# thekingofkings/embedding

Measured on AMD Instinct MI355X. Metric: SGNS training edges/sec, higher is better.
Workload: dtype f32

## Files before the change

### embedding_amd/_native.py

```python
import ctypes as C
import os

_HERE = os.path.dirname(os.path.abspath(__file__))
LIB_PATH = os.path.join(_HERE, "libdge.so")

DGE_OK, DGE_ERR_ARG, DGE_ERR_RANGE, DGE_ERR_TOPK, DGE_ERR_CAP, DGE_ERR_STATE, DGE_ERR_DEVICE, DGE_ERR_IO = range(8)


class DgeError(RuntimeError):
    def __init__(self, code, msg):
        super().__init__("libdge error %d: %s" % (code, msg))
        self.code = code


class TrainConfig(C.Structure):
    _fields_ = [
        ("dim", C.c_int32), ("window", C.c_int32), ("negative", C.c_int32), ("min_count", C.c_int32),
        ("epochs", C.c_int32), ("workers", C.c_int32), ("alpha", C.c_float), ("min_alpha", C.c_float),
        ("seed", C.c_uint64), ("table_size", C.c_int64), ("n_vertices", C.c_int32), ("update_policy", C.c_int32),
        ("use_hs", C.c_int32), ("reserved", C.c_int32),
    ]


class TrainStats(C.Structure):
# ... 55 lines not shown
    "dge_names_add": (_int, [_vp, _vp, _i64]),
    "dge_names_count": (_int, [_vp, _P(_i64)]),
    "dge_names_cstrs": (_int, [_vp, _P(_vp)]),
    "dge_names_free": (None, [_vp]),
    "dge_walks_from_seq_text": (_int, [_int, _vp, _i64, _vp, _int, _P(_vp), _P(SeqInfo)]),
    "dge_walks_from_seq_files": (_int, [_int, _vp, _i32, _vp, _int, _P(_vp), _P(SeqInfo)]),
    "dge_walks_to_seq_text": (_int, [_vp, _i64, _i64, _vp, _int, _vp, _i64, _P(_i64), _P(SeqOutInfo)]),
    "dge_walks_write_seq": (_int, [_vp, _i64, _i64, _vp, _int, C.c_char_p, _int, _P(SeqOutInfo)]),
    "dge_walks_to_host": (_int, [_vp, _vp, _i64]),
    "dge_walks_info": (_int, [_vp, _P(_i64), _P(_i32), _P(_vp)]),
    "dge_walks_add_position_prefix": (_int, [_vp, _i32]),
    "dge_walks_free": (None, [_vp]),
    "dge_count_tokens": (_int, [_vp, _i64, _i64, _i32, _vp]),
    "dge_model_create": (_int, [_int, _P(TrainConfig), _vp, _P(_vp)]),
    "dge_model_set_stream": (_int, [_vp, _vp]),
    "dge_model_train": (_int, [_vp, _vp, _i64, _i64, _i64, _i32, _i64, _dbl, _i64]),
    "dge_train_sgns": (_int, [_int, _vp, _i64, _i32, _P(TrainConfig), _P(_vp)]),
    "dge_train_sgns_device": (_int, [_vp, _P(TrainConfig), _P(_vp)]),
    "dge_model_walk_and_train": (_int, [_vp, _vp, _vp, _i64, _i64, _i64, _i64, _i32, _i64, _dbl, _i64]),
    "dge_model_vectors": (_int, [_vp, _P(_vp), _P(_vp), _P(_i64), _P(_i32)]),
    "dge_model_syn1neg": (_int, [_vp, _P(_vp)]),
    "dge_model_syn1": (_int, [_vp, _P(_vp), _P(_i64)]),
    "dge_model_huffman": (_int, [_vp, _P(_vp), _P(_vp), _P(_vp)]),
    "dge_model_counts": (_int, [_vp, _P(_vp)]),
    "dge_model_table": (_int, [_vp, _P(_vp), _P(_i64)]),
    "dge_model_stats": (_int, [_vp, _P(TrainStats)]),
    "dge_model_row_rates": (_int, [_vp, _P(C.c_double), _P(C.c_double), _P(C.c_double), _P(C.c_double)]),
    "dge_model_table_placement": (_int, [_vp, _i32, _vp, _vp, _vp]),
    "dge_model_table_runs": (_int, [_vp, _vp, _vp]),
    "dge_model_tune_placement": (_int, [_vp, _vp, _i64, _i64, _i32, _vp, _vp, _vp]),
    "dge_model_placement_search": (_int, [_vp, _vp, _vp, _vp, _vp]),
    "dge_model_reset_stats": (_int, [_vp]),
    "dge_model_schedule": (_int, [_vp, _P(_i32), _P(_i64), _P(_i32)]),
    "dge_model_kernel": (_int, [_vp, C.c_char_p, _i32]),
    "dge_model_lock_stats": (_int, [_vp, _P(_i64), _P(_i64), _P(_i64)]),
    "dge_model_score_pairs": (_int, [_vp, _vp, _vp, _i64, _vp]),
    "dge_model_eval_links": (_int, [_vp, _vp, _i64, _i64, _i32, C.c_uint64, _P(EvalResult)]),
    "dge_model_eval_sgns": (_int, [_vp, _vp, _i64, _i64, C.c_uint64, _P(EvalResult)]),
    "dge_write_vec": (_int, [_vp, _vp, C.c_char_p, _int]),
    "dge_model_free": (None, [_vp]),
    "dge_model_set_partition": (_int, [_vp, _i32, _i32, _i32]),
    "dge_model_partition_floats": (_int, [_vp, _i32, _P(_i64)]),
    "dge_model_export_partition": (_int, [_vp, _int, _i32, _i32, _vp]),
    "dge_model_import_partition": (_int, [_vp, _int, _i32, _i32, _vp]),
    "dge_model_export_partition_async": (_int, [_vp, _int, _i32, _i32, _vp, _vp]),
    "dge_model_import_partition_async": (_int, [_vp, _int, _i32, _i32, _vp, _vp]),
    "dge_model_stream": (_int, [_vp, _P(_vp)]),
    "dge_host_sync_count": (_int, [_P(_i64)]),
    "dge_model_sync_size": (_int, [_vp, _P(_i64)]),
    "dge_model_snapshot": (_int, [_vp]),
    "dge_model_export_delta": (_int, [_vp, _vp]),
    "dge_model_import_delta": (_int, [_vp, _vp, C.c_float]),
    "dge_comm_unique_id": (_int, [_vp]),
    "dge_comm_create": (_int, [_P(_vp), _vp, _int, _int, _int]),
    "dge_comm_free": (None, [_vp]),
    "dge_model_allreduce_deltas": (_int, [_vp, _vp]),
    "dge_model_ring_pass": (_int, [_vp, _vp, _i32]),
    "dge_model_gather_table": (_int, [_vp, _vp, _int]),
    "dge_set_tuning": (_int, [_i32, _i64]),
    "dge_get_tuning": (_int, [_i32, _vp]),
    "dge_ndcg_at_k": (_int, [_int, _vp, _i32, _vp, _i32, _i32, _i32, _P(_dbl), _P(_dbl)]),
    "dge_knn_cosine": (_int, [_int, _vp, _i32, _i32, _i32, _vp, _vp, _P(_dbl)]),
    "dge_vectors_from_vec_text": (_int, [_int, _vp, _i64, _int, _vp, _int, _P(_vp), _P(VecInfo)]),
    "dge_vectors_from_vec_files": (_int, [_int, _vp, _i32, _int, _vp, _int, _P(_vp), _P(VecInfo)]),
    "dge_vectors_from_host": (_int, [_int, _vp, _i64, _i32, _vp, _P(_vp)]),
    "dge_vectors_info": (_int, [_vp, _P(_i64), _P(_i32), _P(_vp), _P(_vp)]),
# ... 50 lines not shown
```

### embedding_amd/csrc/sgns.hip

```cpp
#include <hipcub/hipcub.hpp>
#include <math.h>
#include <stdlib.h>
#include <string.h>

#include <algorithm>
#include <limits>
#include <string>

#include "dge_algos.h"
#include "dge_internal.h"
#include "sgns_kernels.h"
#include "sgns_model.h"

std::atomic<int64_t> g_dge_tuning[DGE_TUNE_COUNT];
namespace { struct TuningInit { TuningInit() { for (auto& k : g_dge_tuning) k.store(-1); } } g_tuning_init; }
std::atomic<int64_t> g_dge_host_syncs{0};
extern "C" int dge_host_sync_count(int64_t* n) {
    if (!n) DGE_FAIL(DGE_ERR_ARG, "dge_host_sync_count: null output");
    *n = g_dge_host_syncs.load(std::memory_order_relaxed);
    return DGE_OK;
}
extern "C" int dge_set_tuning(int32_t knob, int64_t value) {
    if (knob < 0 || knob >= DGE_TUNE_COUNT) DGE_FAIL(DGE_ERR_ARG, "dge_set_tuning: unknown knob %d", knob);
    g_dge_tuning[knob] = value < 0 ? -1 : value;
// ... 554 lines not shown
    dge_model* m = const_cast<dge_model*>(mc);
    if (!m || !out) DGE_FAIL(DGE_ERR_ARG, "dge_model_stats: null argument");
    int rc = dge_drain_events(m);
    if (rc) return rc;
    unsigned long long c[4] = {0, 0, 0, 0};
    DGE_HIP(hipMemcpy(c, m->d_counters, sizeof(c), hipMemcpyDeviceToHost));
    out->pairs = (int64_t)c[0]; out->words = (int64_t)c[1];
    out->kernel_ms = m->kernel_ms; out->walk_kernel_ms = m->walk_ms; out->launches = m->launches;
    if (c[3]) {
        DGE_HIP(hipMemsetAsync(m->d_counters + 3, 0, sizeof(unsigned long long), m->stream));
        DGE_HIP(hipStreamSynchronize(m->stream));
        DGE_FAIL(DGE_ERR_STATE, "a training launch was ended by its watchdog: %llu workers waited for row locks beyond the launch's time budget and left their walks untrained "
                 "(update_policy %d on this vocabulary: use 0 (auto) or 7)", c[3], m->cfg.update_policy);
    }
    return DGE_OK;
}

extern "C" int dge_model_table_runs(const dge_model* m, int32_t* n_runs, int32_t* n_exceptions) {
    if (!m) DGE_FAIL(DGE_ERR_ARG, "dge_model_table_runs: null model");
    if (n_runs) *n_runs = m->n_runs;
    if (n_exceptions) *n_exceptions = m->n_exc;
    return DGE_OK;
}

extern "C" int dge_model_schedule(const dge_model* m, int32_t* update_policy, int64_t* workers, int32_t* hot_rows) {
    if (!m) DGE_FAIL(DGE_ERR_ARG, "dge_model_schedule: null model");
    if (!m->has_plan) DGE_FAIL(DGE_ERR_STATE, "dge_model_schedule: nothing has been trained yet");
    if (update_policy) *update_policy = m->last_plan.reported_policy();
    if (workers) *workers = m->last_plan.workers;
    if (hot_rows) *hot_rows = m->last_plan.hot_rows;
    return DGE_OK;
}

extern "C" int dge_model_lock_stats(const dge_model* mc, int64_t* pairs_put_back, int64_t* rounds_short, int64_t* rounds) {
    dge_model* m = const_cast<dge_model*>(mc);
    if (!m) DGE_FAIL(DGE_ERR_ARG, "dge_model_lock_stats: null model");
    DGE_HIP(hipSetDevice(m->device));
    DGE_HIP(hipStreamSynchronize(m->stream));
    unsigned long long c[3] = {0, 0, 0};
    DGE_HIP(hipMemcpy(c, m->d_counters + 4, sizeof(c), hipMemcpyDeviceToHost));
    if (pairs_put_back) *pairs_put_back = (int64_t)c[0];
    if (rounds_short) *rounds_short = (int64_t)c[1];
    if (rounds) *rounds = (int64_t)c[2];
    return DGE_OK;
}

extern "C" int dge_model_kernel(const dge_model* m, char* buf, int32_t cap) {
    if (!m || !buf || cap <= 0) DGE_FAIL(DGE_ERR_ARG, "dge_model_kernel: bad argument");
    if (!m->has_plan) DGE_FAIL(DGE_ERR_STATE, "dge_model_kernel: nothing has been trained yet");
    snprintf(buf, (size_t)cap, "%s", m->last_plan.kernel_name().c_str());
    return DGE_OK;
}

extern "C" int dge_model_reset_stats(dge_model* m) {
    if (!m) DGE_FAIL(DGE_ERR_ARG, "dge_model_reset_stats: null model");
    int rc = dge_drain_events(m);
    if (rc) return rc;
    DGE_HIP(hipMemsetAsync(m->d_counters, 0, 2 * sizeof(unsigned long long), m->stream));
    DGE_HIP(hipMemsetAsync(m->d_counters + 4, 0, 3 * sizeof(unsigned long long), m->stream));
    DGE_HIP(hipStreamSynchronize(m->stream));
    m->kernel_ms = 0; m->walk_ms = 0; m->launches = 0;
    return DGE_OK;
}

extern "C" int dge_model_set_partition(dge_model* m, int32_t n_parts, int32_t ctx_part, int32_t tgt_part) {
    if (!m) DGE_FAIL(DGE_ERR_ARG, "dge_model_set_partition: null model");
// ... 7 lines not shown
```

### embedding_amd/csrc/sgns_kernels.h

```cpp
#pragma once
#include <hip/hip_runtime.h>
#include <stdint.h>

#include "dge_algos.h"
#include "dge_internal.h"
#include "sgns_plan.h"

#define EXP_TABLE_SIZE 1000
#define MAX_EXP 6
#define NEG_BATCH 5

struct TrainParams {
    const int32_t* sen; const int64_t* len; const int64_t* wb;
    float* syn0; float* syn1neg;
    int32_t acc_rows, acc_drain;
    const uint4* ctab;
    const double* run_base; const uint32_t* run_row; const uint32_t* exc_slot; const int32_t* exc_row;
    int32_t n_runs, n_exc;
    double T_inv;
    const float* exp_table;
    int64_t n_rows; int32_t L, W, K, stride;
    int32_t D;
    int64_t V, T;
    uint64_t T_magic, W_magic;
// ... 1150 lines not shown
            l1.v[q].x += neu.v[q].x; l1.v[q].y += neu.v[q].y; l1.v[q].z += neu.v[q].z; l1.v[q].w += neu.v[q].w;
        }
        if (HOTMIX && (last < hot_rows || p.syn0_free)) {
            if (use_mb) lk_post<DCH>(s_mb, s_mb_flag, wk, n_posts, 2, lane == 0 ? last : -1, 1.0f, neu, lane);
            else rowA_atomic_axpy<DCH>(syn0, last, lane, 1.0f, neu);
        } else {
            rowA_store<DCH, 16, BIG>(l1, syn0, last, lane);
            row_commit_wait(STRICT ? row_probe_lines(syn0, last, lane, DCH * 2) : 0.f);
            if (lane == 14) row_unlock<STRICT>(locks0, last);
        }
        my_pairs++;
        if (PART) {
            pair_mask &= pair_mask - 1ull;
            c = first_bit_from(pair_mask, 0, c_hi + 1);
        } else {
            c++;
            if (c == i) c++;
        }
    }
    LK_CLOSE_CENTRE();
    if (pend_row >= 0 && !flushA_blocking<DCH, STRICT, BIG, HOTMIX>(syn1neg, locks1, pend_row, my_dh + (cur_buf ^ 1) * DCH * 64 + lane, lane, hot_rows, WD ? &s_deadline : nullptr)) LK_GIVE_UP();
#undef LK_TOK
#undef LK_POSITIVE
#undef LK_CLOSE_CENTRE
#undef LK_GIVE_UP
    if (lane == 0) {
        if (my_pairs) atomicAdd(&p.counters[0], my_pairs);
        if (my_words) atomicAdd(&p.counters[1], my_words);
        if (PART) { atomicAdd(&p.counters[4], (unsigned long long)n_aborted); atomicAdd(&p.counters[5], (unsigned long long)n_short); atomicAdd(&p.counters[6], (unsigned long long)n_rounds); }
        if (use_mb) __hip_atomic_fetch_add(&s_mb_done, 1, __ATOMIC_RELEASE, __HIP_MEMORY_SCOPE_WORKGROUP);
    }
}

#define HSW_NQ (DCH <= 2 ? 6 : 3)
template <int DCH>
__device__ __forceinline__ void hot_addA(float* s_hot, int* s_cnt, int slot, int drain, const TableView& t, int32_t row, int lane, const Row<DCH>& x) {
    float* a = s_hot + slot * (DCH * 64) + 4 * lane;
#pragma unroll
    for (int c = 0; c < DCH; c++) {
        atomicAdd(a + c * 64 + 0, x.v[c].x); atomicAdd(a + c * 64 + 1, x.v[c].y); atomicAdd(a + c * 64 + 2, x.v[c].z); atomicAdd(a + c * 64 + 3, x.v[c].w);
    }
    int n = 0;
    if (lane == 0) n = atomicAdd(&s_cnt[slot], 1) + 1;
    n = __shfl(n, 0, 16);
    if (n % drain == 0) {
        float* e = s_hot + slot * (DCH * 64) + lane;
        float* gp = t.base + (size_t)row * (t.row_bytes / 4) + lane;
#pragma unroll
        for (int c = 0; c < DCH; c++)
#pragma unroll
            for (int m = 0; m < 4; m++) {
                if ((uint32_t)(c * 64 + 16 * m + lane) >= t.valid) continue;
                const float v = atomicExch(e + c * 64 + 16 * m, 0.f);
                if (v != 0.f) atomicAdd(gp + c * 64 + 16 * m, v);
            }
    }
}
template <int DCH>
__device__ __forceinline__ void row_add(Row<DCH>& y, const Row<DCH>& x) {
#pragma unroll
    for (int c = 0; c < DCH; c++) { y.v[c].x += x.v[c].x; y.v[c].y += x.v[c].y; y.v[c].z += x.v[c].z; y.v[c].w += x.v[c].w; }
}
__device__ __forceinline__ int hsw_n_copies(const TrainParams& p, int32_t nd) {
    int r = 1;
#pragma unroll
    for (int k = 1; k < HS_REP; k++) r += nd >= p.hs_rep_thr[k] ? 1 : 0;
// ... 477 lines not shown
            if (pl.hs) {
                if (pl.part) hipLaunchKernelGGL((k_sgns_train<DCH, 2, BIG, true, true>), g, b, pl.shmem, st, p);
                else hipLaunchKernelGGL((k_sgns_train<DCH, 2, BIG, true, false>), g, b, pl.shmem, st, p);
            } else if (pl.part) hipLaunchKernelGGL((k_sgns_train<DCH, 2, BIG, false, true>), g, b, 0, st, p);
            else hipLaunchKernelGGL((k_sgns_train<DCH, 2, BIG, false, false>), g, b, 0, st, p);
            break;
        case TrainForm::HsCentre:
            if constexpr (DCH <= 4 && !BIG) {
                if (!pl.nlock) hipLaunchKernelGGL((k_sgns_train_hsw<DCH, false, 3>), g, b, pl.shmem, st, p);
                else if (pl.waves == 3) {
                    if (pl.head) hipLaunchKernelGGL((k_sgns_train_hsw<DCH, true, 3, true>), g, b, pl.shmem, st, p);
                    else hipLaunchKernelGGL((k_sgns_train_hsw<DCH, true, 3>), g, b, pl.shmem, st, p);
                } else if constexpr (DCH <= 2) {
                    if (pl.head) {
                        (void)hipFuncSetAttribute((const void*)k_sgns_train_hsw<DCH, true, 7, true>, hipFuncAttributeMaxDynamicSharedMemorySize, (int)pl.shmem);
                        hipLaunchKernelGGL((k_sgns_train_hsw<DCH, true, 7, true>), g, b, pl.shmem, st, p);
                    } else {
                        (void)hipFuncSetAttribute((const void*)k_sgns_train_hsw<DCH, true, 7>, hipFuncAttributeMaxDynamicSharedMemorySize, (int)pl.shmem);
                        hipLaunchKernelGGL((k_sgns_train_hsw<DCH, true, 7>), g, b, pl.shmem, st, p);
                    }
                }
            }
            break;
        case TrainForm::Locked:
            if (pl.hotmix) {
                if (pl.part) hipLaunchKernelGGL((k_sgns_train_locked<DCH, false, BIG, true, true>), g, b, 0, st, p);
                else hipLaunchKernelGGL((k_sgns_train_locked<DCH, false, BIG, true, false>), g, b, 0, st, p);
            } else if (pl.part) {
                if (pl.wdog) hipLaunchKernelGGL((k_sgns_train_locked<DCH, false, BIG, false, true, true>), g, b, 0, st, p);
                else hipLaunchKernelGGL((k_sgns_train_locked<DCH, false, BIG, false, true>), g, b, 0, st, p);
            } else if (pl.strict) {
                if (pl.wdog) hipLaunchKernelGGL((k_sgns_train_locked<DCH, true, BIG, false, false, true>), g, b, 0, st, p);
                else hipLaunchKernelGGL((k_sgns_train_locked<DCH, true, BIG, false, false>), g, b, 0, st, p);
            } else {
                if (pl.wdog) hipLaunchKernelGGL((k_sgns_train_locked<DCH, false, BIG, false, false, true>), g, b, 0, st, p);
                else hipLaunchKernelGGL((k_sgns_train_locked<DCH, false, BIG, false, false>), g, b, 0, st, p);
            }
            break;
        default: break;
    }
}
template <int DCH>
static inline void launch_train(const TrainParams& p, const TrainPlan& pl, hipStream_t st) {
    if (pl.big) launch_train_b<DCH, true>(p, pl, st);
    else launch_train_b<DCH, false>(p, pl, st);
}
```

### embedding_amd/csrc/sgns_plan.h

```cpp
#pragma once
#include <math.h>
#include <stdarg.h>
#include <stdint.h>
#include <stdio.h>

#include <algorithm>
#include <string>
#include <vector>

#include "../../include/dge.h"

#define HS_REP 16
#define HS_REP_NODES 64
#define HS_REP_ROWS ((HS_REP - 1) * HS_REP_NODES)
#ifndef DGE_LOCKED_WAVES
#define DGE_LOCKED_WAVES 3
#endif
#ifndef DGE_HOTMIX_WAVES
#define DGE_HOTMIX_WAVES 3
#endif
#ifndef DGE_HS_WAVES
#define DGE_HS_WAVES 3
#endif

static inline double dge_expected_pairs_per_walk(int L, int W) {
    double e = 0.0;
    for (int i = 0; i < L; i++)
        for (int r = 1; r <= W; r++) e += (double)(std::min(L - 1, i + r) - std::max(0, i - r)) / (double)W;
    return e;
}

struct ScheduleStats {
    int64_t V = 0;
    int32_t D = 0, stride = 0;
    int64_t total_words = 0;
    double neg_norm = 1.0;
    double neg_collision = 1.0;
    double row_share_max = 1.0;
    int64_t hot_rows_auto = 0;
    int64_t hot_rows_serial = 0;
    int32_t hs_rep_auto = 0;
    int32_t hs_rep_thr32[32] = {0};
    int32_t hs_cold_auto = 0;
    int n_cus = 256;
};

static inline ScheduleStats schedule_stats(const int64_t* counts, int64_t V, int32_t D, int32_t stride, int n_cus) {
    ScheduleStats s;
    s.V = V; s.D = D; s.stride = stride; s.n_cus = n_cus;
    int64_t tw = 0;
    for (int64_t i = 0; i < V; i++) tw += counts[i];
    s.total_words = tw;
// ... 70 lines not shown
    if (row_share_caps_workers(s)) return 2;
    if (locks_work(s)) return s.hot_rows_serial > 0 ? 7 : 5;
    if (s.V >= 131072 && s.hot_rows_auto <= s.V / 4) return 7;
    return 2;
}

static inline bool small_rows(const dge_train_config& cfg, const ScheduleStats& s, int policy, int part_n, int32_t L, bool big, const int64_t* knob) {
    return policy == 2 && cfg.use_hs == 0 && part_n <= 1 && cfg.dim > 16 && cfg.dim <= 32 && s.stride == 64 && L <= 64 && !big && knob[DGE_TUNE_SMALL_ROWS] != 0;
}

enum class TrainForm { Sorted, InOrder, RowRmw, Atomics, SmallRows, Locked, HsCentre };

struct TrainPlan {
    TrainForm form = TrainForm::InOrder;
    bool hs = false;
    bool part = false;
    bool strict = false;
    bool hotmix = false;
    bool wdog = false;
    bool nlock = false;
    bool head = false;
    int waves = 0;
    bool big = false;
    int64_t workers = 0;
    unsigned blocks = 0, threads = 0;
    size_t shmem = 0;
    int32_t hot_rows = 0, acc_rows = 0, acc_drain = 16, syn0_free = 0;
    int32_t hs_hot0 = 0x7fffffff, hs_n_hot = 0, hs_drain = 1, hs_cold = 0, hs_wave = 0, hs_rep0 = 0x7fffffff, hs_rep_n = 0;
    int32_t hs_rep_thr[HS_REP] = {0x7fffffff, 0x7fffffff, 0x7fffffff, 0x7fffffff, 0x7fffffff, 0x7fffffff, 0x7fffffff, 0x7fffffff,
                                  0x7fffffff, 0x7fffffff, 0x7fffffff, 0x7fffffff, 0x7fffffff, 0x7fffffff, 0x7fffffff, 0x7fffffff};
    uint64_t wd_ticks = 0;
    bool runs_off = false;
    bool walk_counter = false;
    char error[512] = "";

    int reported_policy() const {
        switch (form) {
            case TrainForm::Sorted: return 8;
            case TrainForm::InOrder: return 0;
            case TrainForm::RowRmw: return 1;
            case TrainForm::Locked: return hotmix ? 7 : (strict ? 6 : 5);
            case TrainForm::HsCentre: return nlock ? (head ? 7 : 5) : 2;
            default: return 2;
        }
    }
    std::string kernel_name() const {
        const std::string blk = part ? ", one block" : "";
        switch (form) {
            case TrainForm::Sorted:
                return part ? "k_sorted_phase (owner-computes, one block of the multi-GPU schedule: k_block_emit + 2 item sorts + 2 phases)"
                            : "k_sorted_phase (owner-computes: k_sorted_emit + 2 item sorts + 2 phases)";
            case TrainForm::HsCentre:
                if (!nlock) return "k_sgns_train_hsw<atomics, 3 waves> (hierarchical softmax, a wave per centre)";
                return std::string("k_sgns_train_hsw<negatives under commit locks") + (head ? ", head rows by atomics" : "") + (waves == 7 ? ", 7 waves>" : ", 3 waves>") +
                       " (hierarchical softmax, a wave per centre)";
            case TrainForm::Locked: return std::string("k_sgns_train_locked<") + (strict ? "strict" : "relaxed") + (hotmix ? ", head rows by atomics" : "") + blk + ">";
            case TrainForm::SmallRows: return "k_sgns_train_small<atomics, 32 lanes a worker>";
            default:
                return std::string("k_sgns_train<") + (form == TrainForm::Atomics ? "atomics" : (form == TrainForm::RowRmw ? "row rmw" : "in-order")) +
                       (hs ? ", hierarchical softmax pair by pair" : "") + blk + ">";
        }
    }
};

static inline int plan_fail(TrainPlan* out, int code, const char* fmt, ...) __attribute__((format(printf, 3, 4)));
static inline int plan_fail(TrainPlan* out, int code, const char* fmt, ...) {
// ... 151 lines not shown
            P.hs_cold = (int32_t)std::min<int64_t>(cold_knob >= 0 ? cold_knob : (int64_t)s.hs_cold_auto, P.hs_rep0);
        } else {
            const int64_t row_b = (int64_t)s.stride * 4 + 4;
            P.hs_n_hot = (int32_t)std::min<int64_t>(std::max<int64_t>(s.V - 1, 0), (hot_kb > 0 ? std::min<int64_t>(hot_kb, nw == 7 ? 100 : 30) * 1024 : (nw == 7 ? 15360 : 30720)) / row_b);
            P.hs_hot0 = (int32_t)(std::max<int64_t>(s.V - 1, 0) - P.hs_n_hot);
            P.hs_cold = (int32_t)std::min<int64_t>(cold_knob >= 0 ? cold_knob : (int64_t)s.hs_cold_auto, P.hs_hot0);
            P.shmem = (size_t)P.hs_n_hot * (size_t)row_b;
        }
    }
    if (P.form == TrainForm::Atomics && hs && workers > 1 && (knob[DGE_TUNE_HS_WAVE] > 0 || (knob[DGE_TUNE_HS_WAVE] < 0 && s.V >= 65536))) {
        P.hs_wave = 1;
        if (workers_auto) workers = std::max<int64_t>(std::min<int64_t>(workers / 16 * 12, (int64_t)s.n_cus * DGE_HS_WAVES * 12), 2);
        P.blocks = (unsigned)((workers + 11) / 12);
    }
    if (P.form == TrainForm::Locked && P.hotmix && workers > 1) {
        if (workers_auto) workers = std::max<int64_t>(workers / 16 * 12, 2);
        P.blocks = (unsigned)((workers + 11) / 12);
        if (part) P.acc_drain = knob[DGE_TUNE_ACC_DRAIN] > 0 ? (int32_t)std::min<int64_t>(knob[DGE_TUNE_ACC_DRAIN], 1 << 20)
                                                             : (int32_t)std::max<int64_t>(1, std::min<int64_t>(8, 2048 / std::max(P.blocks, 1u)));
    }
    P.workers = workers;
    P.big = big;
    const bool in_order = P.form == TrainForm::InOrder && !hs && !part;
    P.walk_counter = workers > 1 && n_rows >= 32 * workers && !in_order && !(knob[DGE_TUNE_STATIC_WALKS] > 0);
    P.runs_off = s.hot_rows_serial > 0 && workers > 1;
    {
        const double bytes = launch_pairs * 8.0 * (double)s.stride * (double)(cfg.negative + 2);
        double budget_s = 5.0 + 100.0 * bytes / 8e12;
        if (knob[DGE_TUNE_WATCHDOG_MS] > 0) budget_s = (double)knob[DGE_TUNE_WATCHDOG_MS] * 1e-3;
        const bool forced_locks = cfg.update_policy == 5 || cfg.update_policy == 6;
        P.wd_ticks = (!forced_locks || knob[DGE_TUNE_WATCHDOG_MS] == 0) ? 0ull : (uint64_t)(budget_s * 1e8);
    }
    P.wdog = P.form == TrainForm::Locked && !P.hotmix && P.wd_ticks != 0;
    if (small && P.form == TrainForm::Atomics && (workers > 1 || knob[DGE_TUNE_SMALL_ROWS] > 0)) {
        P.form = TrainForm::SmallRows;
        P.threads = 256u; P.blocks = (unsigned)((workers * 32 + 255) / 256);
    }
    return DGE_OK;
}
```

### embedding_amd/engine.py

```python
import ctypes as C
import os

import numpy as np

from ._native import EvalResult, SeqInfo, SeqOutInfo, TrainConfig, TrainStats, VecInfo, check, lib


def _ptr(a):
    return a.ctypes.data_as(C.c_void_p) if a is not None else None


def _dev_ptr(t):
    if t is None:
        return None
    if isinstance(t, int):
        return C.c_void_p(t)
    return C.c_void_p(t.data_ptr())


class DeviceGraph:

    def __init__(self, device=0):
        h = C.c_void_p(0)
        check(lib.dge_graph_create(C.byref(h), int(device)))
# ... 474 lines not shown
    def _eval_dict(r):
        return dict(pairs=r.pairs, negatives=r.negatives, skipped=r.skipped, auc=r.auc, loss=r.loss, kernel_ms=r.kernel_ms)

    def eval_links(self, corpus, regions_per_slice, seed=3, row0=0, n_rows=None):
        if n_rows is None:
            n_rows = corpus.shape[0] - row0
        r = EvalResult()
        check(lib.dge_model_eval_links(self._h, corpus._h, int(row0), int(n_rows), int(regions_per_slice), int(seed), C.byref(r)))
        return self._eval_dict(r)

    def eval_sgns(self, corpus, seed=3, row0=0, n_rows=None):
        if n_rows is None:
            n_rows = corpus.shape[0] - row0
        r = EvalResult()
        check(lib.dge_model_eval_sgns(self._h, corpus._h, int(row0), int(n_rows), int(seed), C.byref(r)))
        return self._eval_dict(r)

    def write_vec(self, path, names=None, header=False):
        arr = None
        if isinstance(names, Names):
            arr = names._cstrs()
        elif names is not None:
            arr = (C.c_char_p * len(names))(*[n.encode() if n is not None else None for n in names])
        check(lib.dge_write_vec(self._h, arr, str(path).encode(), int(bool(header))))

    def load_vectors(self, v):
        n = C.c_int64(0)
        check(lib.dge_model_load_vectors(self._h, v._h, C.byref(n)))
        return n.value

    def schedule(self):
        pol, w, hot = C.c_int32(0), C.c_int64(0), C.c_int32(0)
        check(lib.dge_model_schedule(self._h, C.byref(pol), C.byref(w), C.byref(hot)))
        return {"update_policy": pol.value, "workers": w.value, "hot_rows": hot.value}

    def lock_stats(self):
        a, b, c = C.c_int64(0), C.c_int64(0), C.c_int64(0)
        check(lib.dge_model_lock_stats(self._h, C.byref(a), C.byref(b), C.byref(c)))
        return {"pairs_put_back": a.value, "rounds_short": b.value, "rounds": c.value}

    def kernel(self):
        buf = C.create_string_buffer(256)
        check(lib.dge_model_kernel(self._h, buf, 256))
        return buf.value.decode()

    def set_partition(self, n_parts, ctx_part=0, tgt_part=0):
        check(lib.dge_model_set_partition(self._h, int(n_parts), int(ctx_part), int(tgt_part)))

    def partition_floats(self, n_parts):
        n = C.c_int64(0); check(lib.dge_model_partition_floats(self._h, int(n_parts), C.byref(n))); return n.value

    def export_partition(self, table, n_parts, part, d_buf):
        check(lib.dge_model_export_partition(self._h, int(table), int(n_parts), int(part), _dev_ptr(d_buf)))

    def import_partition(self, table, n_parts, part, d_buf):
        check(lib.dge_model_import_partition(self._h, int(table), int(n_parts), int(part), _dev_ptr(d_buf)))

    def export_partition_async(self, table, n_parts, part, d_buf, consumer_stream=0):
        check(lib.dge_model_export_partition_async(self._h, int(table), int(n_parts), int(part), _dev_ptr(d_buf), C.c_void_p(int(consumer_stream))))

    def import_partition_async(self, table, n_parts, part, d_buf, producer_stream=0):
        check(lib.dge_model_import_partition_async(self._h, int(table), int(n_parts), int(part), _dev_ptr(d_buf), C.c_void_p(int(producer_stream))))

    def stream(self):
        p = C.c_void_p(0); check(lib.dge_model_stream(self._h, C.byref(p))); return p.value or 0

    def sync_size(self):
# ... 42 lines not shown
```

### include/dge.h

```cpp
#ifndef DGE_H
#define DGE_H
#include <stdint.h>

#ifdef __cplusplus
extern "C" {
#endif

#define DGE_VERSION 106

enum {
    DGE_OK = 0,
    DGE_ERR_ARG = 1,
    DGE_ERR_RANGE = 2,
    DGE_ERR_TOPK = 3,
    DGE_ERR_CAP = 4,
    DGE_ERR_STATE = 5,
    DGE_ERR_DEVICE = 6,
    DGE_ERR_IO = 7
};

typedef struct dge_graph dge_graph;
typedef struct dge_walks dge_walks;
typedef struct dge_model dge_model;

// ... 91 lines not shown
    int64_t pairs;
    int64_t words;
    double  kernel_ms;
    double  walk_kernel_ms;
    int64_t launches;
} dge_train_stats;

int  dge_count_tokens(const dge_walks* w, int64_t row0, int64_t n_rows, int32_t n_vertices, int64_t* d_counts);
int  dge_model_create(int device, const dge_train_config* cfg, const int64_t* d_counts, dge_model** out);
int  dge_model_set_stream(dge_model* m, void* hip_stream);
int  dge_model_train(dge_model* m, const dge_walks* w, int64_t row0, int64_t n_rows, int64_t walk_index_base,
                     int32_t epoch, int64_t words_before, double words_scale, int64_t total_walks_per_epoch);
int  dge_train_sgns(int device, const int32_t* walks , int64_t n_walks, int32_t max_len,
                    const dge_train_config* cfg, dge_model** out);
int  dge_train_sgns_device(const dge_walks* w, const dge_train_config* cfg, dge_model** out);
int  dge_model_walk_and_train(dge_model* m, const dge_graph* g, dge_walks* w, int64_t row0, int64_t n_rows,
                              int64_t walk_seed, int64_t walk_index_base, int32_t epoch, int64_t words_before,
                              double words_scale, int64_t total_walks_per_epoch);
int  dge_model_vectors(dge_model* m, const float** syn0, const int32_t** vocab_ids, int64_t* V, int32_t* dim);
int  dge_model_syn1neg(dge_model* m, const float** syn1neg);
int  dge_model_syn1(dge_model* m, const float** syn1, int64_t* rows);
int  dge_model_huffman(dge_model* m, const int64_t** offsets, const int32_t** points, const uint64_t** codes);
int  dge_model_counts(dge_model* m, const int64_t** counts);
int  dge_model_table(dge_model* m, const int32_t** table, int64_t* table_size);
int  dge_model_stats(const dge_model* m, dge_train_stats* out);
int  dge_model_row_rates(dge_model* m, double* read_gb_per_s, double* rewrite_gb_per_s, double* lock_exchanges_per_s, double* table_lookups_per_s);
int  dge_model_reset_stats(dge_model* m);
int  dge_model_table_placement(const dge_model* m, int32_t table, int32_t* candidates, double* best_gb_per_s, double* worst_gb_per_s);
int  dge_model_table_runs(const dge_model* m, int32_t* n_runs, int32_t* n_exceptions);
int  dge_model_tune_placement(dge_model* m, const dge_walks* w, int64_t row0, int64_t n_rows, int32_t candidates, double* ms_before, double* ms_after,
                              int32_t* arrays_moved);
int  dge_model_placement_search(const dge_model* m, int32_t* runs, double* ms_before, double* ms_after, int32_t* arrays_moved);
int  dge_model_schedule(const dge_model* m, int32_t* update_policy, int64_t* workers, int32_t* hot_rows);
int  dge_model_kernel(const dge_model* m, char* buf, int32_t cap);
int  dge_model_lock_stats(const dge_model* m, int64_t* pairs_put_back, int64_t* rounds_short, int64_t* rounds);
int  dge_host_sync_count(int64_t* n);
typedef struct dge_eval_result {
    int64_t pairs;
    int64_t negatives;
    int64_t skipped;
    double  auc;
    double  loss;
    double  kernel_ms;
} dge_eval_result;

int  dge_model_score_pairs(dge_model* m, const int32_t* d_ctx, const int32_t* d_tgt, int64_t n, float* d_score);

int  dge_model_eval_links(dge_model* m, const dge_walks* w, int64_t row0, int64_t n_rows,
                          int32_t regions_per_slice, uint64_t seed, dge_eval_result* out);

int  dge_model_eval_sgns(dge_model* m, const dge_walks* w, int64_t row0, int64_t n_rows,
                         uint64_t seed, dge_eval_result* out);

int  dge_write_vec(dge_model* m, const char* const* names, const char* path, int header);
void dge_model_free(dge_model* m);

int  dge_model_set_partition(dge_model* m, int32_t n_parts, int32_t ctx_part, int32_t tgt_part);
int  dge_model_partition_floats(const dge_model* m, int32_t n_parts, int64_t* n_floats);
int  dge_model_export_partition(dge_model* m, int table, int32_t n_parts, int32_t part, float* d_buf);
int  dge_model_import_partition(dge_model* m, int table, int32_t n_parts, int32_t part, const float* d_buf);
int  dge_model_export_partition_async(dge_model* m, int table, int32_t n_parts, int32_t part, float* d_buf, void* consumer_stream);
int  dge_model_import_partition_async(dge_model* m, int table, int32_t n_parts, int32_t part, const float* d_buf, void* producer_stream);
int  dge_model_stream(const dge_model* m, void** hip_stream);

int  dge_model_sync_size(const dge_model* m, int64_t* n_floats);
int  dge_model_snapshot(dge_model* m);
// ... 89 lines not shown
```

Measured before the change: 987.9 million.

## Add tiled locked SGNS kernel processing four centres per wave with shared context rows

Adds a new locked-update kernel in which each 64-lane wave is split into four 16-lane groups, each handling a different centre word. When several groups need the same context row, that row is locked and loaded once and shared through LDS, and their gradient contributions are combined before a single store. The planner picks this kernel for non-strict, non-hotmix, non-partitioned locked training with small rows, short walks and few negatives. The aim is fewer lock round-trips and fewer syn0 loads per pair. The cost is extra intra-wave barriers, more LDS use, and a different update order than the existing locked kernel.

```diff
diff --git a/embedding_amd/_native.py b/embedding_amd/_native.py
--- a/embedding_amd/_native.py
+++ b/embedding_amd/_native.py
@@ -111,6 +111,7 @@
     "dge_model_placement_search": (_int, [_vp, _vp, _vp, _vp, _vp]),
     "dge_model_reset_stats": (_int, [_vp]),
     "dge_model_schedule": (_int, [_vp, _P(_i32), _P(_i64), _P(_i32)]),
+    "dge_model_schedule_tile": (_int, [_vp, _P(_i32)]),
     "dge_model_kernel": (_int, [_vp, C.c_char_p, _i32]),
     "dge_model_lock_stats": (_int, [_vp, _P(_i64), _P(_i64), _P(_i64)]),
     "dge_model_score_pairs": (_int, [_vp, _vp, _vp, _i64, _vp]),
diff --git a/embedding_amd/csrc/sgns.hip b/embedding_amd/csrc/sgns.hip
--- a/embedding_amd/csrc/sgns.hip
+++ b/embedding_amd/csrc/sgns.hip
@@ -610,6 +610,13 @@
     return DGE_OK;
 }
 
+extern "C" int dge_model_schedule_tile(const dge_model* m, int32_t* tile) {
+    if (!m || !tile) DGE_FAIL(DGE_ERR_ARG, "dge_model_schedule_tile: null argument");
+    if (!m->has_plan) DGE_FAIL(DGE_ERR_STATE, "dge_model_schedule_tile: nothing has been trained yet");
+    *tile = m->last_plan.tile ? 1 : 0;
+    return DGE_OK;
+}
+
 extern "C" int dge_model_lock_stats(const dge_model* mc, int64_t* pairs_put_back, int64_t* rounds_short, int64_t* rounds) {
     dge_model* m = const_cast<dge_model*>(mc);
     if (!m) DGE_FAIL(DGE_ERR_ARG, "dge_model_lock_stats: null model");
diff --git a/embedding_amd/csrc/sgns_kernels.h b/embedding_amd/csrc/sgns_kernels.h
--- a/embedding_amd/csrc/sgns_kernels.h
+++ b/embedding_amd/csrc/sgns_kernels.h
@@ -1206,6 +1206,261 @@
     }
 }
 
+template <int DCH>
+__global__ void __launch_bounds__(256, DCH == 1 ? 4 : DGE_LOCKED_WAVES)
+k_sgns_train_locked_tile(TrainParams p) {
+    __shared__ float s_exp[EXP_TABLE_SIZE];
+    __shared__ float s_dh[16 * 2 * DCH * 64];
+    __shared__ __attribute__((aligned(16))) float s_l1[4 * DCH * 64];
+    __shared__ double s_run_base[DGE_RUN_MAX];
+    __shared__ uint32_t s_run_row[DGE_RUN_MAX + 1];
+    __shared__ uint32_t s_exc_slot[DGE_RUN_EXC];
+    __shared__ int32_t s_exc_row[DGE_RUN_EXC];
+    const bool use_runs = p.n_runs > 0;
+    if (use_runs) {
+        for (int i = threadIdx.x; i < DGE_RUN_MAX; i += blockDim.x) s_run_base[i] = p.run_base[i];
+        for (int i = threadIdx.x; i < DGE_RUN_MAX + 1; i += blockDim.x) s_run_row[i] = p.run_row[i];
+        for (int i = threadIdx.x; i < DGE_RUN_EXC; i += blockDim.x) { s_exc_slot[i] = p.exc_slot[i]; s_exc_row[i] = p.exc_row[i]; }
+    }
+    for (int i = threadIdx.x; i < EXP_TABLE_SIZE; i += blockDim.x) s_exp[i] = p.exp_table[i];
+    __syncthreads();
+
+    const int lane = threadIdx.x & 15;
+    const int wk = threadIdx.x >> 4;
+    const int grp = wk & 3;
+    const int gsh = threadIdx.x & 48;
+    const int64_t wave = (int64_t)blockIdx.x * (blockDim.x >> 6) + __builtin_amdgcn_readfirstlane((int)(threadIdx.x >> 6));
+    const int64_t n_waves = p.n_workers >> 2;
+    if (wave >= n_waves) return;
+
+    TableView syn0 = make_view(p.syn0, p.V, p.stride, 0);
+    TableView syn1neg = make_view(p.syn1neg, p.V, p.stride, 0);
+    syn0.valid = syn1neg.valid = (uint32_t)p.D;
+    int* const locks1 = p.locks;
+    int* const locks0 = p.locks + p.V + 1;
+
+    uint64_t mA = 1, cA = 0;
+    for (int j = 0; j <= lane; j++) { mA *= DGE_W2V_MULT; cA = cA * DGE_W2V_MULT + 11; }
+
+    const int L = p.L, W = p.W, K = p.K;
+    unsigned long long my_pairs = 0, my_words = 0;
+    int64_t w_next = wave;
+    int32_t word = 0;
+    Row<DCH> h;
+    bool h_dirty = false;
+    int32_t pend_row = -1;
+    int cur_buf = 0;
+    float* const my_dh = s_dh + (size_t)wk * 2 * DCH * 64;
+    float4* const my_l1 = reinterpret_cast<float4*>(s_l1 + (size_t)(wk >> 2) * DCH * 64) + lane;
+
+#define LKT_POSITIVE()                                                                                                 \
+    do {                                                                                                               \
+        const float f_ = row_dot(l1, h);                                                                               \
+        const float g_ = sgns_g(f_, 1.0f, alpha, s_exp);                                                               \
+        row_axpy(neu, g_, h);                                                                                          \
+        row_axpy(h, g_, l1);                                                                                           \
+        float* d_ = my_dh + cur_buf * DCH * 64 + lane;                                                                 \
+        _Pragma("unroll") for (int q_ = 0; q_ < DCH; q_++) {                                                           \
+            d_[q_ * 64] = fmaf(g_, l1.v[q_].x, d_[q_ * 64]); d_[q_ * 64 + 16] = fmaf(g_, l1.v[q_].y, d_[q_ * 64 + 16]); \
+            d_[q_ * 64 + 32] = fmaf(g_, l1.v[q_].z, d_[q_ * 64 + 32]); d_[q_ * 64 + 48] = fmaf(g_, l1.v[q_].w, d_[q_ * 64 + 48]); \
+        }                                                                                                              \
+        h_dirty = true;                                                                                                \
+    } while (0)
+#define LKT_WAVE_ORDER() do { __builtin_amdgcn_fence(__ATOMIC_ACQ_REL, "wavefront"); __builtin_amdgcn_wave_barrier(); } while (0)
+#define LKT_SHARE_L1()                                                                                                 \
+    do {                                                                                                               \
+        if (share_l1) {                                                                                                \
+            share_l1 = false;                                                                                          \
+            if (lead) { _Pragma("unroll") for (int q_ = 0; q_ < DCH; q_++) my_l1[q_ * 16] = l1.v[q_]; }                \
+            LKT_WAVE_ORDER();                                                                                          \
+            if (!lead) { _Pragma("unroll") for (int q_ = 0; q_ < DCH; q_++) l1.v[q_] = my_l1[q_ * 16]; }               \
+            LKT_WAVE_ORDER();                                                                                          \
+        }                                                                                                              \
+    } while (0)
+
+    for (;;) {
+        const int64_t w = w_next;
+        if (w >= p.n_rows) break;
+        {
+            unsigned long long t = 0;
+            if ((threadIdx.x & 63) == 0) t = atomicAdd(p.next_walk, 1ull);
+            const uint32_t lo = (uint32_t)__builtin_amdgcn_readfirstlane((int)(uint32_t)t), hi = (uint32_t)__builtin_amdgcn_readfirstlane((int)(uint32_t)(t >> 32));
+            w_next = (int64_t)(((uint64_t)hi << 32) | lo) + n_waves;
+        }
+        const int len = (int)p.len[w];
+        if (len <= 0) continue;
+        if (grp == 0) my_words += (unsigned long long)len;
+        const int32_t* sen = p.sen + w * L;
+        const int32_t tk0 = lane < L ? sen[lane] : -1;
+        const int32_t tk1 = lane + 16 < L ? sen[lane + 16] : -1;
+        const int32_t tk2 = lane + 32 < L ? sen[lane + 32] : -1;
+        const int32_t tk3 = lane + 48 < L ? sen[lane + 48] : -1;
+#define LKT_TOK(idx) walk_tok(true, sen, (idx), tk0, tk1, tk2, tk3)
+        const int64_t done = p.words_done_base + (p.words_scale == 1.0 ? p.wb[w] : (int64_t)((double)p.wb[w] * p.words_scale));
+        float alpha = (float)((double)p.alpha0 * (1.0 - (double)done / (double)(p.all_words + 1)));
+        if (alpha < p.min_alpha) alpha = p.min_alpha;
+        const int64_t gbase = (p.gidx_base + w) * (int64_t)L;
+
+        for (int i0 = 0; i0 < len; i0 += 4) {
+            const int i = i0 + grp;
+            const int ic = min(i, len - 1);
+            const int32_t word_i = LKT_TOK(ic);
+            uint64_t s = dge_mix64(p.seed + (uint64_t)(gbase + ic));
+            s = s * DGE_W2V_MULT + 11;
+            const int radius = W - (int)dge_fast_mod(s, (uint64_t)W, p.W_magic);
+            const int lo = max(0, ic - radius), hi = min(len - 1, ic + radius);
+            const bool has_pairs = i < len && hi > lo;
+            if (has_pairs) {
+                word = word_i;
+                if (pend_row == word) {
+                    flushA_blocking<DCH, false, false>(syn1neg, locks1, pend_row, my_dh + (cur_buf ^ 1) * DCH * 64 + lane, lane);
+                    pend_row = -1;
+                }
+                rowA_load<DCH, 16, false>(h, syn1neg, word, lane);
+                float* d = my_dh + cur_buf * DCH * 64 + lane;
+#pragma unroll
+                for (int q = 0; q < DCH; q++) { d[q * 64] = 0.f; d[q * 64 + 16] = 0.f; d[q * 64 + 32] = 0.f; d[q * 64 + 48] = 0.f; }
+            }
+
+            const int c_end = min(len - 1, i0 + 3 + W);
+            for (int c = max(0, i0 - W); c <= c_end; c++) {
+                const bool active = has_pairs && c >= lo && c <= hi && c != i;
+                const unsigned long long act = __ballot(active);
+                if (!act) continue;
+                const int leader = (int)__builtin_ctzll(act) >> 4;
+                const bool lead = grp == leader;
+                const bool multi = (act & (act - 1)) != 0;
+                const int32_t last = LKT_TOK(c);
+
+                int32_t t = -1;
+                {
+                    const uint64_t sl = s * mA + cA;
+                    if (active && lane < K) {
+                        const uint64_t slot = dge_fast_mod(sl >> 16, (uint64_t)p.T, p.T_magic);
+                        t = use_runs ? neg_row_by_runs((uint32_t)slot, s_run_base, s_run_row, s_exc_slot, s_exc_row, p.n_exc, p.T_inv, p.V) : -2;
+                        if (t == -2) t = neg_table_row(p.ctab, slot);
+                        if (t == 0 && p.V > 1) t = (int32_t)(sl % (uint64_t)(p.V - 1)) + 1;
+                        if (t == word) t = -1;
+                    }
+                    const uint64_t s_moved = K > 0 ? shfl16_u64(sl, K - 1) : s;
+                    if (active) s = s_moved;
+                }
+                unsigned pend13 = (unsigned)(__ballot(active && lane < K && t >= 0) >> gsh) & 0x1FFFu;
+                if (lane == 13) t = pend_row;
+                if (lane == 14) t = last;
+                bool flush_pending = active && pend_row >= 0;
+
+                Row<DCH> l1, neu;
+                row_zero(neu);
+                bool have_l1 = false, l1_only = false;
+                while (!have_l1 || __ballot(pend13 != 0)) {
+                    const bool others_ok = have_l1 || !l1_only;
+                    const bool want = (others_ok && lane < K && ((pend13 >> lane) & 1u) && !(flush_pending && t == pend_row)) ||
+                                      (others_ok && lane == 13 && flush_pending) || (lead && lane == 14 && !have_l1);
+                    const bool won = want ? row_trylock(lane == 14 ? locks0 : locks1, t) : false;
+                    const unsigned long long bal = __ballot(won);
+                    const unsigned gotl = (unsigned)(bal >> gsh) & 0xFFFFu;
+                    if (!have_l1 && !((bal >> (leader * 16 + 14)) & 1ull)) {
+                        if (won) row_unlock<false>(locks1, t);
+                        l1_only = true;
+                        __builtin_amdgcn_s_sleep(8);
+                        continue;
+                    }
+                    const bool got_l1 = !have_l1;
+                    const unsigned got13 = gotl & 0x1FFFu & pend13;
+                    const bool gotf = flush_pending && ((gotl >> 13) & 1u);
+                    Row<DCH> fr;
+                    if (got_l1) rowA_load<DCH, 16, false>(l1, syn0, (lead && ((gotl >> 14) & 1u)) ? last : p.filler_row, lane);
+                    if (__ballot(flush_pending)) rowA_load<DCH, 16, false>(fr, syn1neg, gotf ? pend_row : p.filler_row, lane);
+                    have_l1 = true;
+                    bool share_l1 = got_l1 && multi;
+                    bool do_pos = got_l1 && active;
+                    for (int base = 0; base < K; base += NEG_BATCH) {
+                        const unsigned got = (got13 >> base) & ((1u << NEG_BATCH) - 1u);
+                        if (!__ballot(got != 0)) continue;
+                        int32_t tg[NEG_BATCH];
+                        Row<DCH> rr[NEG_BATCH];
+#pragma unroll
+                        for (int q = 0; q < NEG_BATCH; q++) tg[q] = __shfl(t, (base + q) & 15, 16);
+#pragma unroll
+                        for (int q = 0; q < NEG_BATCH; q++) rowA_load<DCH, 16, false>(rr[q], syn1neg, ((got >> q) & 1u) ? tg[q] : p.filler_row, lane);
+                        LKT_SHARE_L1();
+                        if (do_pos) { do_pos = false; LKT_POSITIVE(); }
+#pragma unroll
+                        for (int q = 0; q < NEG_BATCH; q++)
+                            if ((got >> q) & 1u) {
+                                float f = row_dot(l1, rr[q]);
+                                float g = sgns_g(f, 0.0f, alpha, s_exp);
+                                row_axpy(neu, g, rr[q]);
+                                row_axpy(rr[q], g, l1);
+                                rowA_store<DCH, 16, false>(rr[q], syn1neg, tg[q], lane);
+                            }
+                    }
+                    LKT_SHARE_L1();
+                    if (do_pos) LKT_POSITIVE();
+                    if (gotf) {
+                        const float* d = my_dh + (cur_buf ^ 1) * DCH * 64 + lane;
+#pragma unroll
+                        for (int q = 0; q < DCH; q++) {
+                            fr.v[q].x += d[q * 64]; fr.v[q].y += d[q * 64 + 16]; fr.v[q].z += d[q * 64 + 32]; fr.v[q].w += d[q * 64 + 48];
+                        }
+                        rowA_store<DCH, 16, false>(fr, syn1neg, pend_row, lane);
+                    }
+                    row_commit_wait(0.f);
+                    if (won && lane != 14) row_unlock<false>(locks1, t);
+                    pend13 &= ~got13;
+                    if (gotf) { flush_pending = false; pend_row = -1; if (lane == 13) t = -1; }
+                    if (__ballot(pend13 != 0)) __builtin_amdgcn_s_sleep(2);
+                }
+
+                if (multi) {
+#pragma unroll
+                    for (int g2 = 0; g2 < 4; g2++) {
+                        if (!((act >> (16 * g2)) & 1ull)) continue;
+                        if (grp == g2) {
+#pragma unroll
+                            for (int q = 0; q < DCH; q++) {
+                                float4 a = my_l1[q * 16];
+                                a.x += neu.v[q].x; a.y += neu.v[q].y; a.z += neu.v[q].z; a.w += neu.v[q].w;
+                                my_l1[q * 16] = a;
+                            }
+                        }
+                        LKT_WAVE_ORDER();
+                    }
+                    if (lead) {
+#pragma unroll
+                        for (int q = 0; q < DCH; q++) l1.v[q] = my_l1[q * 16];
+                    }
+                } else {
+#pragma unroll
+                    for (int q = 0; q < DCH; q++) {
+                        l1.v[q].x += neu.v[q].x; l1.v[q].y += neu.v[q].y; l1.v[q].z += neu.v[q].z; l1.v[q].w += neu.v[q].w;
+                    }
+                }
+                if (lead) rowA_store<DCH, 16, false>(l1, syn0, last, lane);
+                row_commit_wait(0.f);
+                if (lead && lane == 14) row_unlock<false>(locks0, last);
+                if (active) my_pairs++;
+            }
+
+            if (h_dirty) {
+                h_dirty = false;
+                if (pend_row >= 0) flushA_blocking<DCH, false, false>(syn1neg, locks1, pend_row, my_dh + (cur_buf ^ 1) * DCH * 64 + lane, lane);
+                pend_row = word; cur_buf ^= 1;
+            }
+        }
+#undef LKT_TOK
+    }
+    if (pend_row >= 0) flushA_blocking<DCH, false, false>(syn1neg, locks1, pend_row, my_dh + (cur_buf ^ 1) * DCH * 64 + lane, lane);
+#undef LKT_POSITIVE
+#undef LKT_SHARE_L1
+#undef LKT_WAVE_ORDER
+    if (lane == 0) {
+        if (my_pairs) atomicAdd(&p.counters[0], my_pairs);
+        if (my_words) atomicAdd(&p.counters[1], my_words);
+    }
+}
+
 #define HSW_NQ (DCH <= 2 ? 6 : 3)
 template <int DCH>
 __device__ __forceinline__ void hot_addA(float* s_hot, int* s_cnt, int slot, int drain, const TableView& t, int32_t row, int lane, const Row<DCH>& x) {
@@ -1749,6 +2004,8 @@
             } else if (pl.strict) {
                 if (pl.wdog) hipLaunchKernelGGL((k_sgns_train_locked<DCH, true, BIG, false, false, true>), g, b, 0, st, p);
                 else hipLaunchKernelGGL((k_sgns_train_locked<DCH, true, BIG, false, false>), g, b, 0, st, p);
+            } else if (pl.tile) {
+                if constexpr (DCH <= 2 && !BIG) hipLaunchKernelGGL((k_sgns_train_locked_tile<DCH>), g, b, 0, st, p);
             } else {
                 if (pl.wdog) hipLaunchKernelGGL((k_sgns_train_locked<DCH, false, BIG, false, false, true>), g, b, 0, st, p);
                 else hipLaunchKernelGGL((k_sgns_train_locked<DCH, false, BIG, false, false>), g, b, 0, st, p);
diff --git a/embedding_amd/csrc/sgns_plan.h b/embedding_amd/csrc/sgns_plan.h
--- a/embedding_amd/csrc/sgns_plan.h
+++ b/embedding_amd/csrc/sgns_plan.h
@@ -18,6 +18,9 @@
 #endif
 #ifndef DGE_HOTMIX_WAVES
 #define DGE_HOTMIX_WAVES 3
+#endif
+#ifndef LK_CHUNK
+#define LK_CHUNK 10
 #endif
 #ifndef DGE_HS_WAVES
 #define DGE_HS_WAVES 3
@@ -154,6 +157,7 @@
     uint64_t wd_ticks = 0;
     bool runs_off = false;
     bool walk_counter = false;
+    bool tile = false;
     char error[512] = "";
 
     int reported_policy() const {
@@ -371,6 +375,8 @@
         P.wd_ticks = (!forced_locks || knob[DGE_TUNE_WATCHDOG_MS] == 0) ? 0ull : (uint64_t)(budget_s * 1e8);
     }
     P.wdog = P.form == TrainForm::Locked && !P.hotmix && P.wd_ticks != 0;
+    P.tile = P.form == TrainForm::Locked && !P.strict && !P.hotmix && !part && !P.wdog && !big && s.stride <= 128 && L <= 64 && cfg.negative <= LK_CHUNK &&
+             P.walk_counter && workers >= 4 && workers % 4 == 0;
     if (small && P.form == TrainForm::Atomics && (workers > 1 || knob[DGE_TUNE_SMALL_ROWS] > 0)) {
         P.form = TrainForm::SmallRows;
         P.threads = 256u; P.blocks = (unsigned)((workers * 32 + 255) / 256);
diff --git a/embedding_amd/engine.py b/embedding_amd/engine.py
--- a/embedding_amd/engine.py
+++ b/embedding_amd/engine.py
@@ -530,7 +530,9 @@
     def schedule(self):
         pol, w, hot = C.c_int32(0), C.c_int64(0), C.c_int32(0)
         check(lib.dge_model_schedule(self._h, C.byref(pol), C.byref(w), C.byref(hot)))
-        return {"update_policy": pol.value, "workers": w.value, "hot_rows": hot.value}
+        tile = C.c_int32(0)
+        check(lib.dge_model_schedule_tile(self._h, C.byref(tile)))
+        return {"update_policy": pol.value, "workers": w.value, "hot_rows": hot.value, "tile": tile.value}
 
     def lock_stats(self):
         a, b, c = C.c_int64(0), C.c_int64(0), C.c_int64(0)
diff --git a/include/dge.h b/include/dge.h
--- a/include/dge.h
+++ b/include/dge.h
@@ -147,6 +147,7 @@
                               int32_t* arrays_moved);
 int  dge_model_placement_search(const dge_model* m, int32_t* runs, double* ms_before, double* ms_after, int32_t* arrays_moved);
 int  dge_model_schedule(const dge_model* m, int32_t* update_policy, int64_t* workers, int32_t* hot_rows);
+int  dge_model_schedule_tile(const dge_model* m, int32_t* tile);
 int  dge_model_kernel(const dge_model* m, char* buf, int32_t cap);
 int  dge_model_lock_stats(const dge_model* m, int64_t* pairs_put_back, int64_t* rounds_short, int64_t* rounds);
 int  dge_host_sync_count(int64_t* n);
```

New measurement: 890.9 million. 0.902x the previous value.
